# jkulhanek/tetra-nerf

Measured on AMD Instinct MI355X. Metric: ray_tet_intersections_per_s, higher is better.
Workload: dtype f32

## Files before the change

### profiles/compare_device_code.py

```python
#!/usr/bin/env python3
import glob
import os
import re
import shutil
import subprocess
import sys
import tempfile

LLVM = os.environ.get("LLVM_BIN", "/opt/rocm/llvm/bin")
FIELDS = (".vgpr_count", ".sgpr_count", ".private_segment_fixed_size", ".group_segment_fixed_size", ".kernarg_segment_size")


def run(*cmd, cwd=None):
    return subprocess.run(cmd, cwd=cwd, check=True, capture_output=True, text=True).stdout


def device_code(so):
    text, blocks = {}, []
    with tempfile.TemporaryDirectory() as tmp:
        shutil.copy(so, os.path.join(tmp, "lib.so"))
        run(f"{LLVM}/llvm-objdump", "--offloading", "lib.so", cwd=tmp)
        for co in sorted(glob.glob(os.path.join(tmp, "*gfx950*"))):
            sym, per_co = None, {}
            for line in run(f"{LLVM}/llvm-objdump", "-d", "--no-show-raw-insn", "--no-leading-addr", co).splitlines():
                m = re.match(r"^<(.+)>:$", line.strip())
                if m:
                    sym = m.group(1)
                    per_co[sym] = []
                elif sym and line.strip() and line.strip() != "...":
                    per_co[sym].append(re.sub(r"\s*//.*$", "", line).strip())
            for k, v in per_co.items():
                text.setdefault(k, set()).add("\n".join(v))
            block = None
            for line in run(f"{LLVM}/llvm-readelf", "--notes", co).splitlines():
                m = re.match(r"^  (- | {2})(\.\w+):\s*(\S+)\s*$", line)
                if not m:
                    continue
                if m.group(1) == "- ":
                    block = {}
                    blocks.append(block)
                if block is not None:
                    block[m.group(2)] = m.group(3)
    meta = {}
    for b in blocks:
        if ".symbol" in b:
            meta.setdefault(b[".symbol"], set()).add(tuple(b.get(f) for f in FIELDS))
    return text, meta


def exported(so):
    return sorted(l.split()[-1] for l in run("nm", "-D", "--defined-only", so).splitlines() if " T tn_" in l)


def main():
    old, new = sys.argv[1:3]
    bad = 0
    eo, en = exported(old), exported(new)
    print(f"exported tn_* names: {len(eo)} / {len(en)}: {'same' if eo == en else 'DIFFERENT'}")
    bad += eo != en
    (to, mo), (tn_, mn) = device_code(old), device_code(new)
    print(f"device symbols: {len(to)} / {len(tn_)}; kernels with notes: {len(mo)} / {len(mn)}")
    for sym in sorted(to):
        if sym not in tn_:
            print("MISSING in new:", sym); bad += 1
        elif to[sym] != tn_[sym]:
            print("TEXT DIFFERS:", sym); bad += 1
    for sym in sorted(set(tn_) - set(to)):
        print("only in new:", sym)
    for k in sorted(mo):
        if mo[k] != mn.get(k):
            print("RESOURCES DIFFER:", k, mo[k], mn.get(k)); bad += 1
    print("identical" if not bad else f"{bad} differences")
    return 1 if bad else 0


if __name__ == "__main__":
    sys.exit(main())
```

### tetra-nerf_amd/csrc/tn_api_tracer.hip

```cpp
#include <algorithm>
#include <cmath>
#include <cstring>
#include <memory>
#include <mutex>

#include "tn_api_common.h"
#include "tn_build.h"
#include "tn_devbuf.h"
#include "tn_kernels.h"

using tn::check_loaded;
using tn::check_pow2_M;
using tn::DeviceGuard;
using tn::guarded;

struct tn_tracer {
    int device = 0;
    std::mutex mu;

    struct Mesh {
        bool loaded = false;
        tn::DeviceMesh view;
        tn::HostMesh host;
        uint32_t bvh_max_stack = 1;
// ... 5 lines not shown
        tn::DevBuf<tn::WalkTet> tets;
        tn::DevBuf<tn::WalkFid> fidt;
        tn::DevBuf<float> hull_nodes, hull_tris;
        tn::RefitTables refit;
        bool device_built = false;
    } mesh;

    struct Options {
        bool gpu_build = true;
        unsigned leaf_width = 16;
        int writer_table = 0;
        bool refit_tables = false;
        int use_walk = 1;
        size_t walk_min_rays = 12288;
        bool walk_min_auto = true;
        bool dense_tails = true;
        bool literal = true;
        size_t log_cap_bytes = 0;
        int spec_fill = 0;
        unsigned spec_k0 = 0;
        tn::FillRange spec{true, 0, true, tn::FillKind::Spans, 512};
        unsigned walk_lds_kb = 26;
        tn::FillRange tail{false, 0, false, tn::FillKind::RowPerBlock, 0};
        unsigned writer_blocks = 0;
        bool hull_flat = true;
        bool small_lds = true;
        unsigned lds_cap = 0;
        unsigned verify_stride = 256;
        bool verify_risk = true;
        unsigned risk_band = 2;
        bool verify_inject = false;
        unsigned literal_sort_passes = 8;
        int cert_ends = 2;
        bool bin_rays = false;
        bool timing = false;
    } opt;

    struct Scratch {
        tn::DevBuf<uint32_t> fallback_list;
        tn::DevBuf<uint32_t> walk_n;
        tn::DevBuf<uint4> hull_entry;
        tn::DevBuf<uint2> literal_list;
        tn::DevBuf<uint4> hit_log;
        tn::DevBuf<uint32_t> verify_list;
        tn::DevBuf<uint32_t> risk_list;
        tn::DevBuf<uint32_t> ray_keys, ray_iota, ray_keys_sorted, order, walk_n_item;
        tn::DevBuf<char> sort_temp;
        static constexpr int N_CTR = 2;
        tn::DevBuf<unsigned long long> stats;
        uint32_t *fallback_count() { return reinterpret_cast<uint32_t *>(stats.p + tn::N_STATS); }
        uint32_t *literal_count() { return fallback_count() + 1; }
        uint32_t *verify_count() { return fallback_count() + 2; }
        uint32_t *risk_count() { return fallback_count() + 3; }
        static constexpr size_t stats_bytes() { return (tn::N_STATS + N_CTR) * sizeof(unsigned long long); }
        size_t last_num_rays = 0;
        bool last_walk = false;
        bool last_binned = false;
        hipStream_t last_stream = nullptr;

        template <typename T>
        static void grow(tn::DevBuf<T> &b, size_t n) { if (b.n < n) b.alloc(n); }
        void reserve(size_t R, size_t log_entries, bool verify, bool risk, size_t sort_temp_bytes = 0) {
            grow(fallback_list, R);
            if (!log_entries) return;
            grow(walk_n, R); grow(literal_list, R); grow(hull_entry, R); grow(hit_log, log_entries);
            if (verify) grow(verify_list, R);
// ... 113 lines not shown
        if (!cap_bytes) {
            size_t free_b = 0, total_b = 0;
            TN_HIP(hipMemGetInfo(&free_b, &total_b));
            cap_bytes = std::min<size_t>((free_b + s().hit_log.n * sizeof(uint4)) / 4, (size_t)24 << 30);
        }
        const size_t chunk = std::max<size_t>(cap_bytes / ((size_t)rows.M * sizeof(uint4)) / 4096 * 4096, 4096);
        return std::min(chunk, R);
    }

    tn::TraceParams trace_params(size_t base, size_t n) const {
        tn::TraceParams q = mesh_params(t, n, rows.at(base), origins + 3 * base, dirs + 3 * base);
        q.stats = s().stats.p;
        q.compact_rows = dense_tails ? 0u : 1u;
        q.sort_passes = o().literal_sort_passes;
        return q;
    }
    tn::WalkParams walk_params(size_t base, size_t n) const {
        const tn::DeviceMesh &m = mesh();
        tn::WalkParams w{};
        w.t = trace_params(base, n);
        w.vars = m.hot;
        w.scene_max = m.bvh.scene_max;
        w.hull_nodes = m.hull_nodes; w.hull_tris = m.hull_tris; w.n_hull_nodes = m.n_hull_nodes; w.n_hull = m.n_hull;
        w.hull_flat = m.hull_nodes + 2 * (size_t)m.n_hull_nodes;
        w.n_hull_leaves = o().hull_flat ? tn::hull_flat_leaves(m.n_hull) : 0u;
        w.n_hull_groups = o().hull_flat ? tn::hull_flat_groups(m.n_hull) : 0u;
        w.ray_base = base;
        w.hull_entry = s().hull_entry.p + base; w.walk_n = s().walk_n.p + base; w.hit_log = s().hit_log.p;
        w.fallback_list = s().fallback_list.p; w.fallback_count = s().fallback_count();
        w.literal_list = o().literal ? s().literal_list.p : nullptr; w.literal_count = s().literal_count();
        w.risk_list = verify_risk() ? s().risk_list.p : nullptr; w.risk_count = s().risk_count();
        w.risk_band = (float)o().risk_band;
        if (binned) { w.order = s().order.p; w.walk_n_item = s().walk_n_item.p; }
        w.cert_ends = o().cert_ends == 2 ? (m.T >= tn::WALK_TET_MIN_TETS ? 1u : 3u) : (uint32_t)o().cert_ends;
        return w;
    }
    tn::WriteParams write_params(size_t base, size_t n) const {
        const tn::Rows r = rows.at(base);
        tn::WriteParams q{};
        q.num_rays = n; q.M = r.M; q.dense_tails = dense_tails ? 1u : 0u;
        q.walk_n = s().walk_n.p + base;
        q.hit_log = s().hit_log.p;
        q.cold = mesh().cold; q.tets = mesh().tets;
        q.out_cells = r.cells; q.out_bary = r.bary; q.out_dist = r.dist; q.out_verts = r.verts;
        if (binned) { q.walk_n = s().walk_n_item.p; q.order = s().order.p; }
        return q;
    }

    void fill_tails(size_t base, size_t n, uint32_t k_hi) const {
        if (!dense_tails) return;
        tn::FillRange f = o().tail;
        f.k_split = k_hi;
        tn::launch_fill(rows.at(base), n, s().walk_n.p + base, f, stream);
    }
    void pair_literal(size_t base, size_t n, hipStream_t st) const {
        if (!o().literal) return;
        tn::launch_postprocess_log(trace_params(base, n), mesh().fidt, s().hit_log.p, s().literal_list.p, s().literal_count(), n, st,
                                   binned ? s().order.p : nullptr);
    }
    void trace_listed(const uint32_t *list, const uint32_t *count, size_t max_items, hipStream_t st) const {
        tn::TraceParams q = trace_params(0, max_items);
        q.ray_list = list; q.item_count = count;
        tn::launch_trace_general(q, st);
    }

    uint32_t spec_fill_first_slot() const {
// ... 548 lines not shown
        std::lock_guard<std::mutex> lock(t->mu);
        tn_tracer::Options &o = t->opt;
        auto set_grid = [](tn::FillRange &f, int v) {
            f.kind = v == -2 ? tn::FillKind::Linear : v < 0 ? tn::FillKind::RowPerBlock : tn::FillKind::Spans;
            f.blocks = v > 0 ? (unsigned)v : 0u;
        };
        const std::string k = name ? name : "";
        if (k == "gpu_build") o.gpu_build = value != 0;
        else if (k == "bin_rays") o.bin_rays = value != 0;
        else if (k == "timing") { o.timing = value != 0; t->sched.tev_valid = false; }
        else if (k == "leaf_width") {
            if (value != 16 && value != 32 && value != 64) throw tn::Error("leaf_width must be 16, 32 or 64");
            o.leaf_width = (unsigned)value;
        }
        else if (k == "walk") o.use_walk = value < 0 ? 0 : (value > 2 ? 2 : value);
        else if (k == "walk_min_rays") { o.walk_min_rays = value < 0 ? 0 : (size_t)value; o.walk_min_auto = false; }
        else if (k == "dense_tails") o.dense_tails = value != 0;
        else if (k == "literal") o.literal = value != 0;
        else if (k == "spec_fill") o.spec_fill = value != 0;
        else if (k == "spec_k0") o.spec_k0 = (unsigned)value;
        else if (k == "spec_blocks") set_grid(o.spec, value);
        else if (k == "hull_flat") o.hull_flat = value != 0;
        else if (k == "writer_blocks") o.writer_blocks = (unsigned)value;
        else if (k == "fill_blocks") set_grid(o.tail, value);
        else if (k == "walk_lds_kb") o.walk_lds_kb = (unsigned)value;
        else if (k == "small_lds") o.small_lds = value != 0;
        else if (k == "lds_cap") {
            if (value < 0 || (value & (value - 1)) != 0 || (value && value < 8)) throw tn::Error("lds_cap must be 0 or a power of two >= 8");
            o.lds_cap = (unsigned)value;
        }
        else if (k == "writer_table") o.writer_table = value;
        else if (k == "refit_tables") o.refit_tables = value != 0;
        else if (k == "cert_ends") { if (value < 0 || value > 3) throw tn::Error("cert_ends must be 0 .. 3"); o.cert_ends = value; }
        else if (k == "verify_inject") o.verify_inject = value != 0;
        else if (k == "literal_sort_passes") o.literal_sort_passes = value < 0 ? 0u : (unsigned)value;
        else if (k == "verify_stride") o.verify_stride = value < 0 ? 0u : (unsigned)value;
        else if (k == "verify_risk") o.verify_risk = value != 0;
        else if (k == "risk_band") o.risk_band = value < 1 ? 1u : (unsigned)value;
        else if (k == "log_cap_mb") o.log_cap_bytes = value <= 0 ? 0 : (size_t)value << 20;
        else throw tn::Error("unknown option " + (name ? k : std::string("(null)")));
    });
}

}
```

### tetra-nerf_amd/csrc/tn_device.h

```cpp
#pragma once
#include "tn_common.h"

namespace tn {

struct RayPre {
    int kx, ky, kz;
    float Sx, Sy, Sz;
    float ox, oy, oz;
};

__device__ __forceinline__ float pick(float x, float y, float z, int k) {
    const bool b0 = (k & 1) != 0, b1 = (k & 2) != 0;
    const float lo = b0 ? y : x;
    return b1 ? z : lo;
}

__device__ __forceinline__ RayPre ray_pre(float ox, float oy, float oz, float dx, float dy, float dz) {
    RayPre r;
    int kz = 0;
    float m = fabsf(dx);
    if (fabsf(dy) > m) { kz = 1; m = fabsf(dy); }
    if (fabsf(dz) > m) { kz = 2; }
    int kx = kz + 1; if (kx == 3) kx = 0;
    int ky = kx + 1; if (ky == 3) ky = 0;
// ... 18 lines not shown
    s.x = akx - r.Sx * akz;
    s.y = aky - r.Sy * akz;
    s.z = r.Sz * akz;
    return s;
}

__device__ __forceinline__ float edge_f(const SV &P, const SV &Q) { return Q.x * P.y - Q.y * P.x; }
__device__ __forceinline__ float edge_d(const SV &P, const SV &Q) {
    return (float)((double)Q.x * (double)P.y - (double)Q.y * (double)P.x);
}

__device__ __forceinline__ bool tri_finish(float U, float V, float W, float Az, float Bz, float Cz,
                                           float &t, float &u, float &v) {
    if ((U < 0.0f || V < 0.0f || W < 0.0f) && (U > 0.0f || V > 0.0f || W > 0.0f)) return false;
    const float det = (U + V) + W;
    if (det == 0.0f) return false;
    const float T = (U * Az + V * Bz) + W * Cz;
    const float tt = T / det;
    if (!(tt > 0.0f && tt < 1e16f)) return false;
    t = tt;
    u = V / det;
    v = W / det;
    return true;
}

__device__ __forceinline__ bool tri_hit_sv(const SV &A, const SV &B, const SV &C, float &t, float &u, float &v) {
    float U = edge_f(B, C), V = edge_f(C, A), W = edge_f(A, B);
    if (U == 0.0f || V == 0.0f || W == 0.0f) {
        U = edge_d(B, C); V = edge_d(C, A); W = edge_d(A, B);
    }
    return tri_finish(U, V, W, A.z, B.z, C.z, t, u, v);
}

__device__ __forceinline__ bool line_box(float ox, float oy, float oz, float ix, float iy, float iz,
                                         float lx, float ly, float lz, float hx, float hy, float hz, float pad) {
    float tn_ = -INFINITY, tf_ = INFINITY;
    {
        const float a = ((lx - ox) - pad) * ix, b = ((hx - ox) + pad) * ix;
        const float mn = a < b ? a : b, mx = a < b ? b : a;
        if (mn > tn_) tn_ = mn;
        if (mx < tf_) tf_ = mx;
    }
    {
        const float a = ((ly - oy) - pad) * iy, b = ((hy - oy) + pad) * iy;
        const float mn = a < b ? a : b, mx = a < b ? b : a;
        if (mn > tn_) tn_ = mn;
        if (mx < tf_) tf_ = mx;
    }
    {
        const float a = ((lz - oz) - pad) * iz, b = ((hz - oz) + pad) * iz;
        const float mn = a < b ? a : b, mx = a < b ? b : a;
        if (mn > tn_) tn_ = mn;
        if (mx < tf_) tf_ = mx;
    }
    const float slack = 4.0f * 1.1920929e-7f * (fabsf(tn_) + fabsf(tf_));
    return (tn_ <= tf_ + slack) || !(tn_ == tn_) || !(tf_ == tf_);
}

__device__ __forceinline__ float safe_inv(float d) {
    if (fabsf(d) < 1e-30f) d = (__float_as_uint(d) >> 31) ? -1e-30f : 1e-30f;
    return 1.0f / d;
}

__device__ __forceinline__ bool common_tet(uint2 a, uint2 b, uint32_t &cell) {
    if (a.x == b.x) { cell = a.x; return true; }
    if (a.x == b.y) { cell = a.x; return true; }
    if (a.y == b.x) { cell = a.y; return true; }
    if (a.y == b.y) { cell = a.y; return true; }
    return false;
}

__device__ __forceinline__ void combine_indices(const uint32_t id1[3], const uint32_t id2[3], float u1, float v1,
                                                float u2, float v2, uint32_t out4[4], float bc1[3], float bc2[3]) {
    out4[0] = 0; out4[1] = id1[0]; out4[2] = id1[1]; out4[3] = id1[2];
    bc1[0] = 1.0f - u1 - v1; bc1[1] = u1; bc1[2] = v1;
    const float ref2[3] = {1.0f - u2 - v2, u2, v2};
    bc2[0] = 0.0f; bc2[1] = 0.0f; bc2[2] = 0.0f;
#pragma unroll
    for (int i = 0; i < 3; ++i) {
        bool was_break = false;
#pragma unroll
        for (int j = 0; j < 3; ++j) {
            if (!was_break && id1[j] == id2[i]) { bc2[j] = ref2[i]; was_break = true; }
        }
        if (!was_break) out4[0] = id2[i];
    }
}

__device__ __forceinline__ uint64_t lanemask_lt() {
// ... 6 lines not shown
```

### tetra-nerf_amd/csrc/tn_kernels.h

```cpp
#pragma once
#include "tn_common.h"
#include "tn_ray_key.h"

namespace tn {

struct Rows {
    uint32_t *num;
    uint32_t *cells;
    float *bary;
    float *dist;
    uint32_t *verts;
    uint32_t M;
    Rows at(size_t base) const {
        return Rows{num ? num + base : nullptr, cells + base * M, bary + base * M * 6, dist + base * M * 2,
                    verts ? verts + base * M * 4 : nullptr, M};
    }
};

struct TraceParams {
    const float *origins;
    const float *dirs;
    const uint32_t *faces;
    const uint32_t *face_tets;
    WideBvh bvh;
// ... 16 lines not shown

void launch_trace_general(const TraceParams &p, hipStream_t stream);
void launch_postprocess_hits(const TraceParams &p, const uint32_t *hit_count, const uint32_t *hit_ids,
                             const float *hit_t, const float *hit_uv, hipStream_t stream);
size_t trace_general_smem_bytes(uint32_t M);
void launch_trace_triangles(const TraceParams &p, uint32_t *out_ids, float *out_t, float *out_uv, uint32_t *out_v3,
                            hipStream_t stream);
void launch_find_tetrahedra(const TraceParams &p, const float *points, uint32_t *out_tet, float *out_bary,
                            uint32_t *out_verts, hipStream_t stream);

void launch_split_walk_records(size_t n4, const WalkVar *vars, WalkHot *hot, WalkCold *cold, WalkTet *tets, WalkFid *fidt, hipStream_t stream);

struct WalkParams {
    TraceParams t;
    const WalkHot *vars;
    float scene_max;
    const float4 *hull_nodes;
    const float4 *hull_tris;
    uint32_t n_hull_nodes;
    const float4 *hull_flat;
    uint32_t n_hull_groups, n_hull_leaves;
    uint32_t n_hull;
    uint4 *hull_entry;
    uint32_t *fallback_list;
    uint32_t *fallback_count;
    uint2 *literal_list;
    uint32_t *literal_count;
    uint32_t *walk_n;
    uint4 *hit_log;
    size_t ray_base;
    uint32_t *risk_list;
    uint32_t *risk_count;
    float risk_band;
    uint32_t cert_ends;
    const uint32_t *order;
    uint32_t *walk_n_item;
};
void launch_trace_walk(const WalkParams &p, hipStream_t stream, size_t lds_reserve = 0);
void launch_postprocess_log(const TraceParams &p, const WalkFid *fidt, const uint4 *hit_log, const uint2 *literal_list,
                            const uint32_t *literal_count, size_t max_items, hipStream_t stream, const uint32_t *order = nullptr);

void launch_verify_counts(const TraceParams &p, uint32_t stride, uint32_t *walk_n, uint32_t *fallback_list, uint32_t *fallback_count,
                          size_t ray_base, hipStream_t stream, bool late = false, bool inject = false, const uint32_t *ray_list = nullptr,
                          const uint32_t *list_count = nullptr, size_t max_list = 0);

struct WriteParams {
    size_t num_rays;
    uint32_t M;
    uint32_t dense_tails;
    const uint32_t *walk_n;
    const uint4 *hit_log;
    const WalkCold *cold;
    const WalkTet *tets;
    uint32_t *out_cells;
    float *out_bary;
    float *out_dist;
    uint32_t *out_verts;
    const uint32_t *order;
};
void launch_write_segments(const WriteParams &q, hipStream_t stream, unsigned max_blocks = 0);
enum class FillKind {
    Spans,
    RowPerBlock,
    Linear,
};
struct FillRange { bool all_rows; uint32_t k_split; bool nontemporal; FillKind kind; unsigned blocks; };
// ... 168 lines not shown
```

### tetra-nerf_amd/csrc/tn_trace_walk.hip

```cpp
#include "tn_device.h"
#include "tn_kernels.h"

#ifndef TN_WALK_DIAG
#define TN_WALK_DIAG 0
#endif
#if TN_WALK_DIAG
__device__ unsigned long long g_walk_diag[16];
__device__ unsigned long long g_walk_time[8];
extern "C" int tn_debug_walk_time(unsigned long long out[8], int reset) {
    if (hipMemcpyFromSymbol(out, HIP_SYMBOL(g_walk_time), sizeof(unsigned long long) * 8) != hipSuccess) return 1;
    if (reset) { unsigned long long z[8] = {}; if (hipMemcpyToSymbol(HIP_SYMBOL(g_walk_time), z, sizeof z) != hipSuccess) return 1; }
    return 0;
}
extern "C" int tn_debug_walk_diag(unsigned long long out[16], int reset) {
    if (hipMemcpyFromSymbol(out, HIP_SYMBOL(g_walk_diag), sizeof(unsigned long long) * 16) != hipSuccess) return 1;
    if (reset) { unsigned long long z[16] = {}; if (hipMemcpyToSymbol(HIP_SYMBOL(g_walk_diag), z, sizeof z) != hipSuccess) return 1; }
    return 0;
}
#endif

namespace tn {

namespace {

// ... 91 lines not shown
        const bool rule_c = vj && cinv_n && cfirst && cn_n == 2u;
        const bool rule_b = vj && !cinv_n && cfirst && cn_n == 3u;
        d2 = d2 || rule_c;
        const uint32_t pend_new_cluster = (0x2810u >> (3u * pend)) & 7u;
        const uint32_t pend_old = pend;
        pend = vj ? (rule_c ? 3u : (rule_b ? 1u : pend)) : (vn ? pend_new_cluster : pend);
        const uint32_t why = (vj && !good) ? (pend_old >= 2u ? 1u : (long_inv ? 2u : (cfirst ? 5u : (cn_n > 3u ? 3u : 4u)))) : 0u;
        const bool fresh = vn || start;
        prev_cmax = vn ? cmax : prev_cmax;
        cmax = vj ? fmaxf(cmax, ct) : (fresh ? ct : cmax);
        cn = vj ? cn_n : (fresh ? 1u : cn);
        cinv = vj ? cinv_n : (fresh ? false : cinv);
        cfirst = start ? true : (vn ? false : cfirst);
        return why;
    }
    __device__ __forceinline__ bool needs_step(bool valid, bool have_prev, float ct) const {
        return valid && (!have_prev || pend != 0u || !(ct - cmax >= TN_EPS));
    }
    __device__ __forceinline__ void fast(bool valid, float ct) {
        prev_cmax = valid ? cmax : prev_cmax;
        cmax = valid ? ct : cmax;
        cn = valid ? 1u : cn;
        cinv = cinv && !valid;
        cfirst = cfirst && !valid;
    }
    __device__ __forceinline__ bool finish(uint32_t nhits) const {
        return ok && pend == 0u && (!cinv || (!cfirst && cn == 2u && nhits >= 4u));
    }
    __device__ __forceinline__ bool drop2() const { return d2; }
    __device__ __forceinline__ uint32_t end_reason() const { return pend ? 6u : 7u; }
};
}

template <bool BINNED>
__global__ __launch_bounds__(WALK_BLOCK) void k_hull_entry(WalkParams p) {
    const TraceParams &t = p.t;

    const uint32_t nblk = (uint32_t)((t.num_items + WALK_BLOCK - 1) / WALK_BLOCK);
    const uint32_t super = blockIdx.x / (8 * XCD_GROUP), rem = blockIdx.x % (8 * XCD_GROUP);
    const uint32_t lb = super * 8 * XCD_GROUP + (rem & 7) * XCD_GROUP + (rem >> 3);
    if (lb >= nblk) return;
    const size_t ray = (size_t)lb * WALK_BLOCK + threadIdx.x;
    const bool active = ray < t.num_items;
    const size_t rr = active ? (BINNED ? (size_t)p.order[ray] : ray) : 0;

    const float ox = t.origins[3 * rr], oy = t.origins[3 * rr + 1], oz = t.origins[3 * rr + 2];
    const float dx = t.dirs[3 * rr], dy = t.dirs[3 * rr + 1], dz = t.dirs[3 * rr + 2];
    const RayPre rp = ray_pre(ox, oy, oz, dx, dy, dz);

    bool flag = false;
    uint32_t why = 0;

    const float pad = 16.0f * 1.1920929e-7f * (fmaxf(fabsf(ox), fmaxf(fabsf(oy), fabsf(oz))) + p.scene_max);
    const float delta = 0.21875f * pad;
    const float kappa = 8.0f * delta;
    const float kappa2 = p.risk_band * kappa;
    auto edge_band = [&](float e, const SV &X, const SV &Y) -> uint32_t {
        const float len = fabsf(X.x - Y.x) + fabsf(X.y - Y.y), ae = fabsf(e);
        return (ae <= kappa * len ? 1u : 0u) | (ae <= kappa2 * len ? 2u : 0u);
    };
    uint32_t risk = 0;
    uint32_t nhull = 0;
    uint32_t hf0 = TN_EMPTY, hf1 = TN_EMPTY, hc0 = 0, hc1 = 0, he0 = 0, he1 = 0, hs0 = 0, hs1 = 0;
    float ht0 = 0.f, ht1 = 0.f;
    auto hull_face = [&](const SV &A, const SV &B, const SV &C, uint32_t fid, uint32_t rec, uint32_t loc, uint32_t slot) {
        const float U = edge_f(B, C), V = edge_f(C, A), W = edge_f(A, B);
        const bool mixed = (U < 0.0f || V < 0.0f || W < 0.0f) && (U > 0.0f || V > 0.0f || W > 0.0f);
        const float det = (U + V) + W;
        if (!mixed && (U == 0.0f || V == 0.0f || W == 0.0f || det == 0.0f)) { flag = true; why = 1; }
        const uint32_t hb = edge_band(U, B, C) | edge_band(V, C, A) | edge_band(W, A, B);
        if (hb & 1u) { flag = true; why = why ? why : 2u; }
        risk |= (hb >> 1) & 1u;
        const float T = (U * A.z + V * B.z) + W * C.z;
        const float tt = T / det;
        const bool s0 = !mixed && nhull == 0, s1 = !mixed && nhull == 1;
        hf0 = s0 ? fid : hf0; ht0 = s0 ? tt : ht0; hc0 = s0 ? rec : hc0; he0 = s0 ? loc : he0; hs0 = s0 ? slot : hs0;
        hf1 = s1 ? fid : hf1; ht1 = s1 ? tt : ht1; hc1 = s1 ? rec : hc1; he1 = s1 ? loc : he1; hs1 = s1 ? slot : hs1;
        nhull += mixed ? 0u : 1u;
    };
    const float ix = safe_inv(dx), iy = safe_inv(dy), iz = safe_inv(dz);
    if (p.n_hull_leaves) {
        extern __shared__ float4 s_hull[];
        const uint32_t nbox2 = 2u * (p.n_hull_groups + p.n_hull_leaves);
        for (uint32_t i = threadIdx.x; i < nbox2; i += WALK_BLOCK) s_hull[i] = p.hull_flat[i];
        float4 *s_tri = s_hull + nbox2;
        for (uint32_t i = threadIdx.x; i < 3u * p.n_hull; i += WALK_BLOCK) s_tri[i] = p.hull_tris[i];
        __syncthreads();
        const float4 *s_leaf = s_hull + 2u * p.n_hull_groups;
        const float pad2 = 2.0f * pad;
        unsigned long long gm = 0ull;
        if (active)
            for (uint32_t g = 0; g < p.n_hull_groups; ++g) {
                const float4 a = s_hull[2 * g], b = s_hull[2 * g + 1];
                gm |= line_box(ox, oy, oz, ix, iy, iz, a.x, a.y, a.z, b.x, b.y, b.z, pad2) ? 1ull << g : 0ull;
            }
        while (gm) {
            const uint32_t g = (uint32_t)__ffsll((long long)gm) - 1u;
            gm &= gm - 1ull;
            const uint32_t l0 = 8u * g;
            uint32_t lm = 0;
#pragma unroll
            for (uint32_t j = 0; j < 8; ++j) {
                const uint32_t l = l0 + j < p.n_hull_leaves ? l0 + j : p.n_hull_leaves - 1u;
                const float4 a = s_leaf[2 * l], b = s_leaf[2 * l + 1];
                lm |= (l0 + j < p.n_hull_leaves && line_box(ox, oy, oz, ix, iy, iz, a.x, a.y, a.z, b.x, b.y, b.z, pad2)) ? 1u << j : 0u;
            }
            while (lm) {
                const uint32_t l = l0 + (uint32_t)__ffs((int)lm) - 1u;
                lm &= lm - 1u;
                const uint32_t first = __float_as_uint(s_leaf[2 * l].w), cnt = __float_as_uint(s_leaf[2 * l + 1].w);
                const float4 *tp = s_tri + 3u * first;
                const float4 *tq = tp + (cnt > 1u ? 3 : 0);
                const float4 v0 = tp[0], v1 = tp[1], v2 = tp[2], w0 = tq[0], w1 = tq[1], w2 = tq[2];
                hull_face(shear(rp, v0.x, v0.y, v0.z), shear(rp, v1.x, v1.y, v1.z), shear(rp, v2.x, v2.y, v2.z),
                          __float_as_uint(v0.w), __float_as_uint(v1.w), __float_as_uint(v2.w), first);
                if (cnt > 1u)
                    hull_face(shear(rp, w0.x, w0.y, w0.z), shear(rp, w1.x, w1.y, w1.z), shear(rp, w2.x, w2.y, w2.z),
                              __float_as_uint(w0.w), __float_as_uint(w1.w), __float_as_uint(w2.w), first + 1u);
            }
        }
    } else {
        uint32_t i = active ? 0u : p.n_hull_nodes;
        while (i < p.n_hull_nodes) {
            const float4 a = p.hull_nodes[2 * (size_t)i], b = p.hull_nodes[2 * (size_t)i + 1];
            if (!line_box(ox, oy, oz, ix, iy, iz, a.x, a.y, a.z, b.x, b.y, b.z, pad)) { i = __float_as_uint(a.w); continue; }
            const uint32_t leaf = __float_as_uint(b.w);
            if (leaf != TN_EMPTY) {
                const uint32_t first = leaf >> 3, cnt = leaf & 7u;
                for (uint32_t k = 0; k < cnt; ++k) {
                    const float4 *tp = p.hull_tris + 3 * (size_t)(first + k);
                    const float4 v0 = tp[0], v1 = tp[1], v2 = tp[2];
                    hull_face(shear(rp, v0.x, v0.y, v0.z), shear(rp, v1.x, v1.y, v1.z), shear(rp, v2.x, v2.y, v2.z),
                              __float_as_uint(v0.w), __float_as_uint(v1.w), __float_as_uint(v2.w), first + k);
                }
            }
            i = i + 1;
        }
    }
    if (nhull != 0 && nhull != 2) { flag = true; why = 2; }
    if (nhull == 2 && !(ht0 < ht1 || ht1 < ht0)) { flag = true; why = 3; }
    if (!active) { flag = false; nhull = 0; }

    if (active) {
        const bool alive = nhull == 2 && !flag;
        const bool first0 = ht0 < ht1;
        uint4 e;
        e.x = alive ? 4u * (first0 ? hc0 : hc1) + (first0 ? he0 : he1) : 0u;
        e.y = first0 ? hf0 : hf1;
        e.z = (first0 ? hs0 : hs1) | (why << 24) | ((risk & 1u) << 28) | ((flag ? 2u : alive ? 1u : 0u) << 29);
        e.w = __float_as_uint(first0 ? ht1 : ht0);
        p.hull_entry[ray] = e;
    }
}

template <typename Order, bool BINNED>
__global__ __launch_bounds__(WALK_BLOCK) void k_trace_walk(WalkParams p) {
    const TraceParams &t = p.t;
    const int lane = threadIdx.x & 63, wave = threadIdx.x >> 6;
    const uint32_t M = t.M;

    const uint32_t nblk = (uint32_t)((t.num_items + WALK_BLOCK - 1) / WALK_BLOCK);
    const uint32_t super = blockIdx.x / (8 * XCD_GROUP), rem = blockIdx.x % (8 * XCD_GROUP);
    const uint32_t lb = super * 8 * XCD_GROUP + (rem & 7) * XCD_GROUP + (rem >> 3);
    if (lb >= nblk) return;
    const size_t ray = (size_t)lb * WALK_BLOCK + threadIdx.x;
    const bool active = ray < t.num_items;
    const size_t rr = active ? (BINNED ? (size_t)p.order[ray] : ray) : 0;

    const float ox = t.origins[3 * rr], oy = t.origins[3 * rr + 1], oz = t.origins[3 * rr + 2];
    const float dx = t.dirs[3 * rr], dy = t.dirs[3 * rr + 1], dz = t.dirs[3 * rr + 2];
    const RayPre rp = ray_pre(ox, oy, oz, dx, dy, dz);

    bool flag = false;
    uint32_t why = 0;
#if TN_WALK_DIAG
    const unsigned long long tick0 = wall_clock64();
#endif

    const float pad = 16.0f * 1.1920929e-7f * (fmaxf(fabsf(ox), fmaxf(fabsf(oy), fabsf(oz))) + p.scene_max);
    const float delta = 0.21875f * pad;
    const float kappa = 8.0f * delta;
    const uint32_t thin_exp = (__float_as_uint(32.0f * delta) >> 23) & 0xFFu;
    const float kappa2 = p.risk_band * kappa;
    auto edge_band = [&](float e, const SV &X, const SV &Y) -> uint32_t {
        const float len = fabsf(X.x - Y.x) + fabsf(X.y - Y.y), ae = fabsf(e);
        return (ae <= kappa * len ? 1u : 0u) | (ae <= kappa2 * len ? 2u : 0u);
    };
    uint32_t risk = 0;
    const uint4 ent = active ? p.hull_entry[ray] : make_uint4(0u, 0u, 0u, 0u);
    const uint32_t ent_state = ent.z >> 29;
    if (ent_state == 2u) { flag = true; why = (ent.z >> 24) & 15u; }
    risk = (ent.z >> 28) & 1u;
    const size_t gw = (size_t)lb * (WALK_BLOCK / 64) + (size_t)wave;
    const size_t logoff = gw * (size_t)M * 64 + (size_t)lane;
    uint4 *mylog = p.hit_log + logoff;

    bool alive = ent_state == 1u;
    const uint32_t f_in0 = ent.y;
    const float t_out = __uint_as_float(ent.w);
    uint32_t c = alive ? ent.x : 0u;
    SV A = {0.f, 0.f, 0.f}, B = A, C = A;
    if (alive) {
        const float4 *tp = p.hull_tris + 3 * (size_t)(ent.z & 0xFFFFFFu);
        const float4 v0 = tp[0], v1 = tp[1], v2 = tp[2];
        A = shear(rp, v0.x, v0.y, v0.z); B = shear(rp, v1.x, v1.y, v1.z); C = shear(rp, v2.x, v2.y, v2.z);
        if (fabsf(A.x) + fabsf(A.y) < pad || fabsf(B.x) + fabsf(B.y) < pad || fabsf(C.x) + fabsf(C.y) < pad) { flag = true; why = 4; alive = false; }
    }
    float Uc = edge_f(B, C), Vc = edge_f(C, A), Wc = edge_f(A, B);
    bool have_prev = false;
    Order ord;
    float pt = 0.f;
    uint32_t nhits = 0, nshort = 0;
    uint32_t steps = 0;
#if TN_WALK_DIAG
    uint32_t lit_why = 0, n_viol = 0;
#endif
    Var cur = load_var(p.vars, c);
    if (alive && ((cur.code_hi >> 8) & 0xFFu) <= thin_exp) {
        const uint32_t eb0 = edge_band(Uc, B, C) | edge_band(Vc, C, A) | edge_band(Wc, A, B);
        if (eb0 & 1u) { flag = true; why = 8; alive = false; }
        risk |= eb0 & 2u;
    }
    if (alive) {
        float tt, uu, vv;
        if (tri_finish(Uc, Vc, Wc, A.z, B.z, C.z, tt, uu, vv)) {
            ord.step(true, false, 0.f, tt, false, 0u);
            have_prev = true; pt = tt; nhits = 1;
            mylog[0] = make_uint4(__float_as_uint(tt), __float_as_uint(uu), __float_as_uint(vv), f_in0 | (3u << 30));
        }
    }

#if TN_WALK_DIAG
    const unsigned long long tick1 = wall_clock64();
#endif
    while (alive) {
        uint32_t bad = 0;
        const SV P = shear(rp, cur.px, cur.py, cur.pz);
        const float ea = edge_f(P, A), eb = edge_f(P, B), ec = edge_f(P, C);
        bad = (fabsf(P.x) + fabsf(P.y) < pad) ? 4u : bad;
        bad = (!bad && (ea == 0.0f || eb == 0.0f || ec == 0.0f)) ? 5u : bad;
        const bool thin = ((cur.code_hi >> 8) & 0xFFu) <= thin_exp;
        const uint32_t band = edge_band(ea, P, A) | edge_band(eb, P, B) | edge_band(ec, P, C);
        bad = (!bad && thin && (band & 1u)) ? 8u : bad;
        risk |= thin ? (band & 2u) : 0u;
        const bool sa = ea > 0.0f, sb = eb > 0.0f, sc = ec > 0.0f;
        const bool su = Uc > 0.0f, sv = Vc > 0.0f, sw = Wc > 0.0f;
        const bool ha = (sb == su) && (su != sc);
        const bool hb = (sc == sv) && (sv != sa);
        const bool hc = (sa == sw) && (sw != sb);
        const uint32_t hmask = (ha ? 1u : 0u) | (hb ? 2u : 0u) | (hc ? 4u : 0u);
        bad = (!bad && __popc(hmask) != 1) ? 6u : bad;
        const uint32_t x = (__ffs(hmask) - 1) & 3u;
        const uint32_t nb = sel3u(cur.nb0, cur.nb1, cur.nb2, x);
        const bool last = nb == TN_EMPTY;
        const Var nxt = load_var(p.vars, (last || bad) ? c : nb);
        __builtin_amdgcn_sched_barrier(0);

        const bool x0 = (x & 1u) != 0, x1 = (x & 2u) != 0;
        const uint32_t w01 = x0 ? (cur.code_lo >> 12) : cur.code_lo;
        const uint32_t w2 = (cur.code_lo >> 24) | (cur.code_hi << 8);
        const uint32_t code = (x1 ? w2 : w01) & 0xFFFu;
        const SV A2 = selsv(P, A, B, C, code & 3u), B2 = selsv(P, A, B, C, (code >> 2) & 3u), C2 = selsv(P, A, B, C, (code >> 4) & 3u);
        const float U = edge_f(B2, C2), V = edge_f(C2, A2), W = edge_f(A2, B2);
        float ct = 0.f, cu = 0.f, cv = 0.f;
        const bool valid = tri_finish(U, V, W, A2.z, B2.z, C2.z, ct, cu, cv);

        if (__builtin_amdgcn_ballot_w64(ord.needs_step(valid, have_prev, ct)) != 0ull) {
            const uint32_t viol = ord.step(valid, have_prev, pt, ct, ((cur.code_hi >> (16u + x)) & 1u) != 0, nhits);
#if TN_WALK_DIAG
            lit_why = lit_why ? lit_why : viol;
            n_viol += viol ? 1u : 0u;
#else
            (void)viol;
#endif
            nshort += (valid && have_prev && fabsf(pt - ct) < TN_EPS) ? 1u : 0u;
        } else {
            ord.fast(valid, ct);
        }
        bad = (!bad && !valid && have_prev) ? 10u : bad;
        bad = (!bad && valid && nhits >= M - 1) ? 9u : bad;
        {
            const uint32_t slot_k = nhits < M - 1 ? nhits : M - 1;
            mylog[(size_t)slot_k * 64] = make_uint4(__float_as_uint(ct), __float_as_uint(cu), __float_as_uint(cv), c | (x << 30));
        }
        nhits += valid ? 1u : 0u;
        pt = valid ? ct : pt;
        have_prev = have_prev || valid;
        bad = (!bad && last && valid && !(ct == t_out)) ? 11u : bad;
        steps++;
        bad = (!bad && !last && steps > MAX_WALK_STEPS) ? 12u : bad;
        flag = bad != 0;
        why = bad;
        alive = !bad && !last;
        c = nb;
        cur = nxt;
        A = A2; B = B2; C = C2;
        Uc = U; Vc = V; Wc = W;
    }

#if TN_WALK_DIAG
    {
        const unsigned long long tick2 = wall_clock64();
        uint32_t ms = steps;
        for (int off = 32; off; off >>= 1) { const uint32_t o2 = __shfl_xor(ms, off); ms = o2 > ms ? o2 : ms; }
        if (lane == 0) {
            atomicAdd(&g_walk_time[0], 1ull);
            atomicAdd(&g_walk_time[1], tick1 - tick0); atomicAdd(&g_walk_time[2], tick2 - tick1);
            atomicMax(&g_walk_time[3], tick1 - tick0); atomicMax(&g_walk_time[4], tick2 - tick1);
            atomicMax(&g_walk_time[5], (unsigned long long)ms); atomicAdd(&g_walk_time[6], (unsigned long long)ms);
        }
    }
#endif
    const bool order_ok = ord.finish(nhits);
    const bool drop2 = ord.drop2();
    const uint32_t nseg = nhits ? nhits - 1 - nshort - (drop2 ? 1u : 0u) : 0;
    const uint32_t wflag = drop2 ? 1u : 0u;
    if (active) {
        const size_t cray = BINNED ? (size_t)p.order[ray] : ray;
        const uint32_t wn = (flag || !order_ok) ? TN_EMPTY : (nhits | (wflag << 30));
        if constexpr (BINNED) p.walk_n_item[ray] = wn;
        if (flag || (!order_ok && !p.literal_list)) {
            const uint32_t slot = atomicAdd(p.fallback_count, 1u);
            p.fallback_list[slot] = (uint32_t)(p.ray_base + cray);
            if (t.stats) atomicAdd(&t.stats[STAT_REASON + (flag ? why : (uint32_t)REASON_ORDER)], 1ull);
            p.walk_n[cray] = TN_EMPTY;
        } else if (!order_ok) {
#if TN_WALK_DIAG
            atomicAdd(&g_walk_diag[0], 1ull);
            atomicAdd(&g_walk_diag[lit_why ? lit_why : ord.end_reason()], 1ull);
            atomicAdd(&g_walk_diag[9], n_viol == 1 ? 1ull : 0ull);
// ... 286 lines not shown
        tt.orig = v.orig;
        uint32_t perm = 0;
        unsigned long long lo64 = 0;
        uint32_t top = 0;
        for (uint32_t e = 0; e < 4; ++e) {
            for (uint32_t m = 0; m < 3; ++m) {
                uint32_t j = 0;
                for (uint32_t k = 0; k < 4; ++k)
                    if (tt.vert[3 - k] == w[e].vid[m + 1]) j = 3 - k;
                perm |= j << (6 * e + 2 * m);
            }
            const unsigned long long code = (unsigned long long)w[e].code_lo | ((unsigned long long)(w[e].code_hi & 0xFu) << 32);
            const unsigned long long c18 = ((code >> 6) & 63ull) | (((code >> 18) & 63ull) << 6) | (((code >> 30) & 63ull) << 12);
            if (e < 3) lo64 |= c18 << (18 * e);
            else { lo64 |= c18 << 54; top = (uint32_t)(c18 >> 10); }
        }
        tt.perm = perm | (top << 24);
        tt.cmb_lo = (uint32_t)lo64; tt.cmb_hi = (uint32_t)(lo64 >> 32);
        tets[i >> 2] = tt;
    }
}
void launch_split_walk_records(size_t n4, const WalkVar *vars, WalkHot *hot, WalkCold *cold, WalkTet *tets, WalkFid *fidt, hipStream_t stream) {
    if (n4 == 0) return;
    hipLaunchKernelGGL(k_split_walk_records, dim3((unsigned)((n4 + 255) / 256)), dim3(256), 0, stream, n4, vars, hot, cold, tets, fidt);
}

void launch_trace_walk(const WalkParams &p, hipStream_t stream, size_t lds_reserve) {
    if (p.t.num_items == 0) return;
    const uint32_t nblk = (uint32_t)((p.t.num_items + WALK_BLOCK - 1) / WALK_BLOCK);
    const uint32_t unit = 8 * XCD_GROUP;
    const uint32_t grid = (nblk + unit - 1) / unit * unit;
    const size_t need = p.n_hull_leaves ? (size_t)(p.n_hull_groups + p.n_hull_leaves) * 32 + (size_t)p.n_hull * 48 : 0;
    if (need > 64 * 1024 &&
        hipFuncSetAttribute(p.order ? reinterpret_cast<const void *>(&k_hull_entry<true>) : reinterpret_cast<const void *>(&k_hull_entry<false>),
                            hipFuncAttributeMaxDynamicSharedMemorySize,
                            (int)((HULL_FLAT_MAX / 2 + HULL_FLAT_MAX / 16) * 32 + HULL_FLAT_MAX * 48)) != hipSuccess)
        throw Error("k_hull_entry: the device refused " + std::to_string(need) + " bytes of dynamic LDS");
    if (lds_reserve > 64 * 1024) lds_reserve = 64 * 1024;
    if (p.order) {
        hipLaunchKernelGGL(k_hull_entry<true>, dim3(grid), dim3(WALK_BLOCK), need, stream, p);
        if (p.cert_ends == 1u) hipLaunchKernelGGL((k_trace_walk<OrderR6, true>), dim3(grid), dim3(WALK_BLOCK), lds_reserve, stream, p);
        else if (p.cert_ends == 3u) hipLaunchKernelGGL((k_trace_walk<OrderR5e, true>), dim3(grid), dim3(WALK_BLOCK), lds_reserve, stream, p);
        else hipLaunchKernelGGL((k_trace_walk<OrderR5, true>), dim3(grid), dim3(WALK_BLOCK), lds_reserve, stream, p);
        return;
    }
    hipLaunchKernelGGL(k_hull_entry<false>, dim3(grid), dim3(WALK_BLOCK), need, stream, p);
    if (p.cert_ends == 1u) hipLaunchKernelGGL((k_trace_walk<OrderR6, false>), dim3(grid), dim3(WALK_BLOCK), lds_reserve, stream, p);
    else if (p.cert_ends == 3u) hipLaunchKernelGGL((k_trace_walk<OrderR5e, false>), dim3(grid), dim3(WALK_BLOCK), lds_reserve, stream, p);
    else hipLaunchKernelGGL((k_trace_walk<OrderR5, false>), dim3(grid), dim3(WALK_BLOCK), lds_reserve, stream, p);
}

}
```

Baseline: 7.680 billion.

## Add walk_math path: shared-reciprocal division, paired box tests, ping-pong walk state

Adds a default-on walk_math variant of the hull entry and walk kernels. Triangle finish computes one reciprocal of the scaled determinant and reuses it for the three quotients through the div_scale/div_fmas/div_fixup sequence, falling back to plain division when any live lane's scaled denominators differ. Hull box tests are evaluated two at a time using 2-wide float vectors so the compiler can emit packed math. The walk loop is unrolled twice with ping-pong state structs to avoid copying the state each step. The risk is more code and register pressure for the extra template instantiations and the unrolled loop.

After: 7.615 billion. No clear change (-0.8%).

```diff
diff --git a/profiles/compare_device_code.py b/profiles/compare_device_code.py
--- a/profiles/compare_device_code.py
+++ b/profiles/compare_device_code.py
@@ -52,7 +52,38 @@
     return sorted(l.split()[-1] for l in run("nm", "-D", "--defined-only", so).splitlines() if " T tn_" in l)
 
 
+CLASSES = (("v_pk_*", r"v_pk_"), ("v_rcp", r"v_rcp_"), ("v_div_*", r"v_div_"), ("v_fma/fmac", r"v_fma"), ("v_mul_f32", r"v_mul_f32"),
+           ("v_add/sub_f32", r"v_(add|sub|subrev)_f32"), ("v_cndmask", r"v_cndmask"), ("v_cmp*", r"v_cmp"), ("v_mov", r"v_mov_"),
+           ("other VALU", r"v_"), ("SALU", r"s_(?!waitcnt|nop|cbranch|branch|endpgm|barrier)"), ("branches", r"s_c?branch"),
+           ("s_waitcnt", r"s_waitcnt"), ("s_nop", r"s_nop"), ("LDS", r"ds_"), ("global/flat", r"(global|flat|buffer|scratch)_"))
+
+
+def counts(pattern, libs):
+    rx = re.compile(pattern)
+    for so in libs:
+        text, meta = device_code(so)
+        print(f"== {so}")
+        for sym in sorted(k for k in meta if rx.search(k)):
+            base = sym[:-3] if sym.endswith(".kd") else sym
+            for body, res in zip(sorted(text.get(base, [""])), sorted(meta[sym])):
+                c = dict.fromkeys((n for n, _ in CLASSES), 0)
+                total = 0
+                for line in body.splitlines():
+                    op = line.split()[0] if line.split() else ""
+                    for n, r in CLASSES:
+                        if re.match(r, op):
+                            c[n] += 1
+                            total += 1
+                            break
+                valu = sum(v for n, v in c.items() if n.startswith("v_") or n == "other VALU")
+                print(f"{run('c++filt', base).strip()}\n    vgpr {res[0]} sgpr {res[1]} scratch {res[2]}  instructions {total}  VALU {valu}")
+                print("    " + "  ".join(f"{n} {v}" for n, v in c.items()))
+    return 0
+
+
 def main():
+    if sys.argv[1] == "--counts":
+        return counts(sys.argv[2], sys.argv[3:])
     old, new = sys.argv[1:3]
     bad = 0
     eo, en = exported(old), exported(new)
diff --git a/profiles/walk_math_kernel_ab.py b/profiles/walk_math_kernel_ab.py
--- /dev/null
+++ b/profiles/walk_math_kernel_ab.py
@@ -0,0 +1,35 @@
+import importlib, sys
+from pathlib import Path
+import numpy as np
+import torch
+sys.path.insert(0, str(Path(__file__).resolve().parents[1]))
+import bench
+tn = importlib.import_module("tetra-nerf_amd")
+scenes = importlib.import_module("tetra-nerf_amd.scenes")
+dev = torch.device("cuda:0")
+VARIANTS = (("0", 0), ("1", 1), ("0 again", 0))
+CFG = {"C2": (15000, 0, 512), "C4": (45000, 2, 512), "C5": (150000, 3, 512)}
+reps = int(sys.argv[1])
+for name in sys.argv[2:]:
+    npts, seed, M = CFG[name]
+    pts, cells = scenes.random_mesh(npts, seed)
+    tr = tn.TetrahedraTracer(dev)
+    tr.load_tetrahedra(torch.from_numpy(pts).to(dev), torch.from_numpy(cells).to(dev))
+    o, d = bench.frame_rays(scenes, 0, 800, 800) if name != "C5" else scenes.outside_in_rays(1 << 20, 4)
+    o, d = torch.from_numpy(o).to(dev), torch.from_numpy(d).to(dev)
+    tr.set_option("timing", 1)
+    res = {n: [] for n, _ in VARIANTS}
+    for rep in range(reps + 1):
+        for n, v in VARIANTS:
+            tr.set_option("walk_math", v)
+            out = tr.trace_rays(o, d, M)
+            del out
+            if rep:
+                res[n].append(tr.trace_timings()["walk"])
+    tr.set_option("timing", 0)
+    print(f"== {name}: {len(cells)} tets, {len(o)} rays; entry search + walk, ms, {reps} interleaved calls per option")
+    for n, _ in VARIANTS:
+        x = np.array(res[n])
+        print(f"walk_math {n:8s} mean {x.mean():.4f}  median {np.median(x):.4f}  min {x.min():.4f}  max {x.max():.4f}  spread(max-min) {x.max() - x.min():.4f}", flush=True)
+    del tr
+    torch.cuda.empty_cache()
diff --git a/tetra-nerf_amd/csrc/tn_api_tracer.hip b/tetra-nerf_amd/csrc/tn_api_tracer.hip
--- a/tetra-nerf_amd/csrc/tn_api_tracer.hip
+++ b/tetra-nerf_amd/csrc/tn_api_tracer.hip
@@ -61,6 +61,7 @@
         bool verify_inject = false;
         unsigned literal_sort_passes = 8;
         int cert_ends = 2;
+        bool walk_math = true;
         bool bin_rays = false;
         bool timing = false;
     } opt;
@@ -240,6 +241,7 @@
         w.risk_list = verify_risk() ? s().risk_list.p : nullptr; w.risk_count = s().risk_count();
         w.risk_band = (float)o().risk_band;
         if (binned) { w.order = s().order.p; w.walk_n_item = s().walk_n_item.p; }
+        w.walk_math = o().walk_math ? 1u : 0u;
         w.cert_ends = o().cert_ends == 2 ? (m.T >= tn::WALK_TET_MIN_TETS ? 1u : 3u) : (uint32_t)o().cert_ends;
         return w;
     }
@@ -854,6 +856,7 @@
         else if (k == "writer_table") o.writer_table = value;
         else if (k == "refit_tables") o.refit_tables = value != 0;
         else if (k == "cert_ends") { if (value < 0 || value > 3) throw tn::Error("cert_ends must be 0 .. 3"); o.cert_ends = value; }
+        else if (k == "walk_math") o.walk_math = value != 0;
         else if (k == "verify_inject") o.verify_inject = value != 0;
         else if (k == "literal_sort_passes") o.literal_sort_passes = value < 0 ? 0u : (unsigned)value;
         else if (k == "verify_stride") o.verify_stride = value < 0 ? 0u : (unsigned)value;
diff --git a/tetra-nerf_amd/csrc/tn_device.h b/tetra-nerf_amd/csrc/tn_device.h
--- a/tetra-nerf_amd/csrc/tn_device.h
+++ b/tetra-nerf_amd/csrc/tn_device.h
@@ -74,6 +74,43 @@
     return tri_finish(U, V, W, A.z, B.z, C.z, t, u, v);
 }
 
+typedef float f32x2 __attribute__((ext_vector_type(2)));
+
+__device__ __forceinline__ float div_tail(float ns, float ds, float r, bool vcc, float den, float num) {
+    float q = ns * r;
+    const float e1 = __builtin_fmaf(-ds, q, ns);
+    q = __builtin_fmaf(e1, r, q);
+    const float e2 = __builtin_fmaf(-ds, q, ns);
+    return __builtin_amdgcn_div_fixupf(__builtin_amdgcn_div_fmasf(e2, r, q, vcc), den, num);
+}
+
+__device__ __forceinline__ bool tri_finish_rcp1(float U, float V, float W, float Az, float Bz, float Cz,
+                                                float &t, float &u, float &v, bool *took_plain = nullptr) {
+    const bool mixed = (U < 0.0f || V < 0.0f || W < 0.0f) && (U > 0.0f || V > 0.0f || W > 0.0f);
+    const float det = (U + V) + W;
+    const bool live = !mixed && !(det == 0.0f);
+    const float T = (U * Az + V * Bz) + W * Cz;
+    bool ct, cv, cw, unused;
+    const float dT = __builtin_amdgcn_div_scalef(T, det, false, &unused), nT = __builtin_amdgcn_div_scalef(T, det, true, &ct);
+    const float dV = __builtin_amdgcn_div_scalef(V, det, false, &unused), nV = __builtin_amdgcn_div_scalef(V, det, true, &cv);
+    const float dW = __builtin_amdgcn_div_scalef(W, det, false, &unused), nW = __builtin_amdgcn_div_scalef(W, det, true, &cw);
+    const bool same = __float_as_uint(dT) == __float_as_uint(dV) && __float_as_uint(dT) == __float_as_uint(dW);
+    float tt, uu, vv;
+    if (__builtin_amdgcn_ballot_w64(live && !same) == 0ull) {
+        float r = __builtin_amdgcn_rcpf(dT);
+        r = __builtin_fmaf(__builtin_fmaf(-dT, r, 1.0f), r, r);
+        tt = div_tail(nT, dT, r, ct, det, T);
+        uu = div_tail(nV, dT, r, cv, det, V);
+        vv = div_tail(nW, dT, r, cw, det, W);
+    } else {
+        tt = T / det; uu = V / det; vv = W / det;
+        if (took_plain) *took_plain = true;
+    }
+    const bool hit = live && tt > 0.0f && tt < 1e16f;
+    t = hit ? tt : t; u = hit ? uu : u; v = hit ? vv : v;
+    return hit;
+}
+
 __device__ __forceinline__ bool line_box(float ox, float oy, float oz, float ix, float iy, float iz,
                                          float lx, float ly, float lz, float hx, float hy, float hz, float pad) {
     float tn_ = -INFINITY, tf_ = INFINITY;
@@ -97,6 +134,36 @@
     }
     const float slack = 4.0f * 1.1920929e-7f * (fabsf(tn_) + fabsf(tf_));
     return (tn_ <= tf_ + slack) || !(tn_ == tn_) || !(tf_ == tf_);
+}
+
+__device__ __forceinline__ bool line_box_decide(float ax, float bx, float ay, float by, float az, float bz) {
+    float tn_ = -INFINITY, tf_ = INFINITY;
+    {
+        const float mn = ax < bx ? ax : bx, mx = ax < bx ? bx : ax;
+        if (mn > tn_) tn_ = mn;
+        if (mx < tf_) tf_ = mx;
+    }
+    {
+        const float mn = ay < by ? ay : by, mx = ay < by ? by : ay;
+        if (mn > tn_) tn_ = mn;
+        if (mx < tf_) tf_ = mx;
+    }
+    {
+        const float mn = az < bz ? az : bz, mx = az < bz ? bz : az;
+        if (mn > tn_) tn_ = mn;
+        if (mx < tf_) tf_ = mx;
+    }
+    const float slack = 4.0f * 1.1920929e-7f * (fabsf(tn_) + fabsf(tf_));
+    return (tn_ <= tf_ + slack) || !(tn_ == tn_) || !(tf_ == tf_);
+}
+__device__ __forceinline__ uint32_t line_box2(float ox, float oy, float oz, float ix, float iy, float iz,
+                                              f32x2 lx, f32x2 ly, f32x2 lz, f32x2 hx, f32x2 hy, f32x2 hz, float pad) {
+    const f32x2 o_x = {ox, ox}, o_y = {oy, oy}, o_z = {oz, oz}, i_x = {ix, ix}, i_y = {iy, iy}, i_z = {iz, iz}, p = {pad, pad};
+    const f32x2 ax = ((lx - o_x) - p) * i_x, bx = ((hx - o_x) + p) * i_x;
+    const f32x2 ay = ((ly - o_y) - p) * i_y, by = ((hy - o_y) + p) * i_y;
+    const f32x2 az = ((lz - o_z) - p) * i_z, bz = ((hz - o_z) + p) * i_z;
+    return (line_box_decide(ax.x, bx.x, ay.x, by.x, az.x, bz.x) ? 1u : 0u) |
+           (line_box_decide(ax.y, bx.y, ay.y, by.y, az.y, bz.y) ? 2u : 0u);
 }
 
 __device__ __forceinline__ float safe_inv(float d) {
diff --git a/tetra-nerf_amd/csrc/tn_kernels.h b/tetra-nerf_amd/csrc/tn_kernels.h
--- a/tetra-nerf_amd/csrc/tn_kernels.h
+++ b/tetra-nerf_amd/csrc/tn_kernels.h
@@ -72,6 +72,7 @@
     uint32_t *risk_list;
     uint32_t *risk_count;
     float risk_band;
+    uint32_t walk_math;
     uint32_t cert_ends;
     const uint32_t *order;
     uint32_t *walk_n_item;
diff --git a/tetra-nerf_amd/csrc/tn_trace_walk.hip b/tetra-nerf_amd/csrc/tn_trace_walk.hip
--- a/tetra-nerf_amd/csrc/tn_trace_walk.hip
+++ b/tetra-nerf_amd/csrc/tn_trace_walk.hip
@@ -147,7 +147,7 @@
 };
 }
 
-template <bool BINNED>
+template <bool BINNED, bool MATH>
 __global__ __launch_bounds__(WALK_BLOCK) void k_hull_entry(WalkParams p) {
     const TraceParams &t = p.t;
 
@@ -204,21 +204,43 @@
         const float4 *s_leaf = s_hull + 2u * p.n_hull_groups;
         const float pad2 = 2.0f * pad;
         unsigned long long gm = 0ull;
+        [[maybe_unused]] auto box_pair = [&](const float4 *box) -> uint32_t {
+            const float *q = reinterpret_cast<const float *>(box);
+            const f32x2 lx = {q[0], q[8]}, ly = {q[1], q[9]}, lz = {q[2], q[10]}, hx = {q[4], q[12]}, hy = {q[5], q[13]}, hz = {q[6], q[14]};
+            return line_box2(ox, oy, oz, ix, iy, iz, lx, ly, lz, hx, hy, hz, pad2);
+        };
+        if constexpr (MATH) {
+            if (active)
+                for (uint32_t g = 0; g < p.n_hull_groups; g += 2) {
+                    const uint32_t m = box_pair(s_hull + 2 * g) & (g + 1u < p.n_hull_groups ? 3u : 1u);
+                    gm |= (unsigned long long)m << g;
+                }
+        } else {
         if (active)
             for (uint32_t g = 0; g < p.n_hull_groups; ++g) {
                 const float4 a = s_hull[2 * g], b = s_hull[2 * g + 1];
                 gm |= line_box(ox, oy, oz, ix, iy, iz, a.x, a.y, a.z, b.x, b.y, b.z, pad2) ? 1ull << g : 0ull;
             }
+        }
         while (gm) {
             const uint32_t g = (uint32_t)__ffsll((long long)gm) - 1u;
             gm &= gm - 1ull;
             const uint32_t l0 = 8u * g;
             uint32_t lm = 0;
+            if constexpr (MATH) {
+#pragma unroll
+                for (uint32_t j = 0; j < 8; j += 2) {
+                    const uint32_t l = l0 + j < p.n_hull_leaves ? l0 + j : p.n_hull_leaves - 1u;
+                    const uint32_t have = (l0 + j < p.n_hull_leaves ? 1u : 0u) | (l0 + j + 1u < p.n_hull_leaves ? 2u : 0u);
+                    lm |= (box_pair(s_leaf + 2 * l) & have) << j;
+                }
+            } else {
 #pragma unroll
             for (uint32_t j = 0; j < 8; ++j) {
                 const uint32_t l = l0 + j < p.n_hull_leaves ? l0 + j : p.n_hull_leaves - 1u;
                 const float4 a = s_leaf[2 * l], b = s_leaf[2 * l + 1];
                 lm |= (l0 + j < p.n_hull_leaves && line_box(ox, oy, oz, ix, iy, iz, a.x, a.y, a.z, b.x, b.y, b.z, pad2)) ? 1u << j : 0u;
+            }
             }
             while (lm) {
                 const uint32_t l = l0 + (uint32_t)__ffs((int)lm) - 1u;
@@ -268,8 +290,12 @@
     }
 }
 
-template <typename Order, bool BINNED>
+template <typename Order, bool BINNED, bool MATH>
 __global__ __launch_bounds__(WALK_BLOCK) void k_trace_walk(WalkParams p) {
+    auto finish = [](float U, float V, float W, float Az, float Bz, float Cz, float &t, float &u, float &v) -> bool {
+        if constexpr (MATH) return tri_finish_rcp1(U, V, W, Az, Bz, Cz, t, u, v);
+        else return tri_finish(U, V, W, Az, Bz, Cz, t, u, v);
+    };
     const TraceParams &t = p.t;
     const int lane = threadIdx.x & 63, wave = threadIdx.x >> 6;
     const uint32_t M = t.M;
@@ -314,14 +340,17 @@
     const uint32_t f_in0 = ent.y;
     const float t_out = __uint_as_float(ent.w);
     uint32_t c = alive ? ent.x : 0u;
-    SV A = {0.f, 0.f, 0.f}, B = A, C = A;
+    struct WalkState { Var rec; SV A, B, C; float U, V, W; };
+    WalkState s0 = {}, s1 = {};
+    SV &A = s0.A, &B = s0.B, &C = s0.C;
     if (alive) {
         const float4 *tp = p.hull_tris + 3 * (size_t)(ent.z & 0xFFFFFFu);
         const float4 v0 = tp[0], v1 = tp[1], v2 = tp[2];
         A = shear(rp, v0.x, v0.y, v0.z); B = shear(rp, v1.x, v1.y, v1.z); C = shear(rp, v2.x, v2.y, v2.z);
         if (fabsf(A.x) + fabsf(A.y) < pad || fabsf(B.x) + fabsf(B.y) < pad || fabsf(C.x) + fabsf(C.y) < pad) { flag = true; why = 4; alive = false; }
     }
-    float Uc = edge_f(B, C), Vc = edge_f(C, A), Wc = edge_f(A, B);
+    float &Uc = s0.U, &Vc = s0.V, &Wc = s0.W;
+    Uc = edge_f(B, C); Vc = edge_f(C, A); Wc = edge_f(A, B);
     bool have_prev = false;
     Order ord;
     float pt = 0.f;
@@ -330,15 +359,15 @@
 #if TN_WALK_DIAG
     uint32_t lit_why = 0, n_viol = 0;
 #endif
-    Var cur = load_var(p.vars, c);
-    if (alive && ((cur.code_hi >> 8) & 0xFFu) <= thin_exp) {
+    s0.rec = load_var(p.vars, c);
+    if (alive && ((s0.rec.code_hi >> 8) & 0xFFu) <= thin_exp) {
         const uint32_t eb0 = edge_band(Uc, B, C) | edge_band(Vc, C, A) | edge_band(Wc, A, B);
         if (eb0 & 1u) { flag = true; why = 8; alive = false; }
         risk |= eb0 & 2u;
     }
     if (alive) {
         float tt, uu, vv;
-        if (tri_finish(Uc, Vc, Wc, A.z, B.z, C.z, tt, uu, vv)) {
+        if (finish(Uc, Vc, Wc, A.z, B.z, C.z, tt, uu, vv)) {
             ord.step(true, false, 0.f, tt, false, 0u);
             have_prev = true; pt = tt; nhits = 1;
             mylog[0] = make_uint4(__float_as_uint(tt), __float_as_uint(uu), __float_as_uint(vv), f_in0 | (3u << 30));
@@ -348,7 +377,10 @@
 #if TN_WALK_DIAG
     const unsigned long long tick1 = wall_clock64();
 #endif
-    while (alive) {
+    auto step = [&](const WalkState &in, WalkState &out) __attribute__((always_inline)) {
+        const Var &cur = in.rec;
+        const SV &A = in.A, &B = in.B, &C = in.C;
+        const float Uc = in.U, Vc = in.V, Wc = in.W;
         uint32_t bad = 0;
         const SV P = shear(rp, cur.px, cur.py, cur.pz);
         const float ea = edge_f(P, A), eb = edge_f(P, B), ec = edge_f(P, C);
@@ -368,7 +400,7 @@
         const uint32_t x = (__ffs(hmask) - 1) & 3u;
         const uint32_t nb = sel3u(cur.nb0, cur.nb1, cur.nb2, x);
         const bool last = nb == TN_EMPTY;
-        const Var nxt = load_var(p.vars, (last || bad) ? c : nb);
+        out.rec = load_var(p.vars, (last || bad) ? c : nb);
         __builtin_amdgcn_sched_barrier(0);
 
         const bool x0 = (x & 1u) != 0, x1 = (x & 2u) != 0;
@@ -378,7 +410,15 @@
         const SV A2 = selsv(P, A, B, C, code & 3u), B2 = selsv(P, A, B, C, (code >> 2) & 3u), C2 = selsv(P, A, B, C, (code >> 4) & 3u);
         const float U = edge_f(B2, C2), V = edge_f(C2, A2), W = edge_f(A2, B2);
         float ct = 0.f, cu = 0.f, cv = 0.f;
-        const bool valid = tri_finish(U, V, W, A2.z, B2.z, C2.z, ct, cu, cv);
+#if TN_WALK_DIAG
+        bool took_plain = false;
+        bool valid;
+        if constexpr (MATH) valid = tri_finish_rcp1(U, V, W, A2.z, B2.z, C2.z, ct, cu, cv, &took_plain);
+        else valid = tri_finish(U, V, W, A2.z, B2.z, C2.z, ct, cu, cv);
+        if (took_plain && lane == (int)(__ffsll((long long)__builtin_amdgcn_ballot_w64(true)) - 1)) atomicAdd(&g_walk_diag[13], 1ull);
+#else
+        const bool valid = finish(U, V, W, A2.z, B2.z, C2.z, ct, cu, cv);
+#endif
 
         if (__builtin_amdgcn_ballot_w64(ord.needs_step(valid, have_prev, ct)) != 0ull) {
             const uint32_t viol = ord.step(valid, have_prev, pt, ct, ((cur.code_hi >> (16u + x)) & 1u) != 0, nhits);
@@ -408,9 +448,20 @@
         why = bad;
         alive = !bad && !last;
         c = nb;
-        cur = nxt;
-        A = A2; B = B2; C = C2;
-        Uc = U; Vc = V; Wc = W;
+        out.A = A2; out.B = B2; out.C = C2;
+        out.U = U; out.V = V; out.W = W;
+    };
+    if constexpr (MATH) {
+        while (alive) {
+            step(s0, s1);
+            if (!alive) break;
+            step(s1, s0);
+        }
+    } else {
+        while (alive) {
+            step(s0, s1);
+            s0 = s1;
+        }
     }
 
 #if TN_WALK_DIAG
@@ -763,22 +814,21 @@
     const uint32_t grid = (nblk + unit - 1) / unit * unit;
     const size_t need = p.n_hull_leaves ? (size_t)(p.n_hull_groups + p.n_hull_leaves) * 32 + (size_t)p.n_hull * 48 : 0;
     if (need > 64 * 1024 &&
-        hipFuncSetAttribute(p.order ? reinterpret_cast<const void *>(&k_hull_entry<true>) : reinterpret_cast<const void *>(&k_hull_entry<false>),
+        hipFuncSetAttribute(p.order ? (p.walk_math ? reinterpret_cast<const void *>(&k_hull_entry<true, true>) : reinterpret_cast<const void *>(&k_hull_entry<true, false>))
+                                    : (p.walk_math ? reinterpret_cast<const void *>(&k_hull_entry<false, true>) : reinterpret_cast<const void *>(&k_hull_entry<false, false>)),
                             hipFuncAttributeMaxDynamicSharedMemorySize,
                             (int)((HULL_FLAT_MAX / 2 + HULL_FLAT_MAX / 16) * 32 + HULL_FLAT_MAX * 48)) != hipSuccess)
         throw Error("k_hull_entry: the device refused " + std::to_string(need) + " bytes of dynamic LDS");
     if (lds_reserve > 64 * 1024) lds_reserve = 64 * 1024;
-    if (p.order) {
-        hipLaunchKernelGGL(k_hull_entry<true>, dim3(grid), dim3(WALK_BLOCK), need, stream, p);
-        if (p.cert_ends == 1u) hipLaunchKernelGGL((k_trace_walk<OrderR6, true>), dim3(grid), dim3(WALK_BLOCK), lds_reserve, stream, p);
-        else if (p.cert_ends == 3u) hipLaunchKernelGGL((k_trace_walk<OrderR5e, true>), dim3(grid), dim3(WALK_BLOCK), lds_reserve, stream, p);
-        else hipLaunchKernelGGL((k_trace_walk<OrderR5, true>), dim3(grid), dim3(WALK_BLOCK), lds_reserve, stream, p);
-        return;
-    }
-    hipLaunchKernelGGL(k_hull_entry<false>, dim3(grid), dim3(WALK_BLOCK), need, stream, p);
-    if (p.cert_ends == 1u) hipLaunchKernelGGL((k_trace_walk<OrderR6, false>), dim3(grid), dim3(WALK_BLOCK), lds_reserve, stream, p);
-    else if (p.cert_ends == 3u) hipLaunchKernelGGL((k_trace_walk<OrderR5e, false>), dim3(grid), dim3(WALK_BLOCK), lds_reserve, stream, p);
-    else hipLaunchKernelGGL((k_trace_walk<OrderR5, false>), dim3(grid), dim3(WALK_BLOCK), lds_reserve, stream, p);
-}
-
-}
+    auto launch = [&](auto binned, auto math) {
+        constexpr bool BINNED = decltype(binned)::value, MATH = decltype(math)::value;
+        hipLaunchKernelGGL((k_hull_entry<BINNED, MATH>), dim3(grid), dim3(WALK_BLOCK), need, stream, p);
+        if (p.cert_ends == 1u) hipLaunchKernelGGL((k_trace_walk<OrderR6, BINNED, MATH>), dim3(grid), dim3(WALK_BLOCK), lds_reserve, stream, p);
+        else if (p.cert_ends == 3u) hipLaunchKernelGGL((k_trace_walk<OrderR5e, BINNED, MATH>), dim3(grid), dim3(WALK_BLOCK), lds_reserve, stream, p);
+        else hipLaunchKernelGGL((k_trace_walk<OrderR5, BINNED, MATH>), dim3(grid), dim3(WALK_BLOCK), lds_reserve, stream, p);
+    };
+    if (p.order) { if (p.walk_math) launch(std::true_type{}, std::true_type{}); else launch(std::true_type{}, std::false_type{}); }
+    else { if (p.walk_math) launch(std::false_type{}, std::true_type{}); else launch(std::false_type{}, std::false_type{}); }
+}
+
+}
```
